# danspeech/danspeech

Measured on AMD Instinct MI355X. Metric: audio-seconds/sec (RTFx) recognize() on 10 s clips, batch=32, higher is better.
Workload: dtype f32 (two-term fp16 split operands, 3 MFMA products, fp32 accumulate)

## Files before the change

danspeech_amd/csrc/conv1_split.hip:

```cpp
#include "common.h"
#include <algorithm>

namespace dsmi {

namespace {

using f16x8 = __attribute__((ext_vector_type(8))) _Float16;
using f16x4 = __attribute__((ext_vector_type(4))) _Float16;
using f16x2 = __attribute__((ext_vector_type(2))) _Float16;
using u32x4 = __attribute__((ext_vector_type(4))) unsigned int;
constexpr float kLoScale = 2048.f, kLoInv = 1.f / 2048.f;

constexpr int KF = 41, KT = 11, SF = 2, ST = 2, PF = 20, PT = 5, CO = 32;
constexpr int C1NF = 8;
constexpr int C1NT = C1NF * 64;
constexpr int C1TT = 64;
constexpr int ROWS = SF * (C1NF - 1) + KF;
constexpr int WIN = ST * (C1TT - 1) + KT + 5;
constexpr int PITCH = 144;
constexpr int COPY = ROWS * PITCH;
constexpr size_t C1_LDS = (size_t)2 * 2 * COPY * 2;

struct Conv1Args {
    const float* x; const uint16_t* wp; const float* bias; const float* bn_a; const float* bn_b; const int32_t* out_lens;
    float* y; uint16_t* y_sp;
    int B, fi, fo, ti, to, xs, ys;
    unsigned* tile_cnt;
};

template <bool SPLIT_OUT, bool BY_DEMAND = false>
__global__ __launch_bounds__(C1NT, 4) void conv1_f16x3_kernel(Conv1Args p) {
    extern __shared__ __attribute__((aligned(16))) unsigned char c1sm[];
    _Float16* Xs = reinterpret_cast<_Float16*>(c1sm);
    const int tid0 = threadIdx.x;
    const int wv = __builtin_amdgcn_readfirstlane(tid0 >> 6);
    const ConvGrid grid{(p.to + C1TT - 1) / C1TT, (p.fo + C1NF - 1) / C1NF, p.B};
    const int total = conv_total(grid);
    const int label = blockIdx.x & 7;
    volatile int* const tk_lds = reinterpret_cast<volatile int*>(c1sm + C1_LDS);
    auto cnt_add = [&](int l) { return __hip_atomic_fetch_add(p.tile_cnt + l * kDenseCntStride, 1u, __ATOMIC_RELAXED, __HIP_MEMORY_SCOPE_AGENT); };
    auto cnt_peek = [&](int l) { return __hip_atomic_load(p.tile_cnt + l * kDenseCntStride, __ATOMIC_RELAXED, __HIP_MEMORY_SCOPE_AGENT); };
    unsigned dead = 0;
    if (BY_DEMAND) {
        if (tid0 == 0) tk_lds[0] = dense_draw(total, label, dead, cnt_add, cnt_peek, grid.nf);
        __syncthreads();
    }
  for (;;) {
    int tid = tid0;
    if (BY_DEMAND) asm volatile("" : "+v"(tid));
    const int lane = tid & 63, li = lane & 31, hk = lane >> 5;
    ConvTile tile;
    if (BY_DEMAND) {
        const int idx = __builtin_amdgcn_readfirstlane(tk_lds[0]);
        if (idx < 0) break;
        tile = conv_tile_at(grid, idx);
    } else {
        tile = ConvTile{(int)blockIdx.x, (int)blockIdx.y, (int)blockIdx.z};
    }
    const int t0 = tile.tt * C1TT, f0 = tile.ft * C1NF, b = tile.z;
    const int f = f0 + wv;
    const int olen = p.out_lens[b];
    const float *bias = p.bias, *bn_a = p.bn_a, *bn_b = p.bn_b;
    if (BY_DEMAND) asm volatile("" : "+s"(bias), "+s"(bn_a), "+s"(bn_b));
    bool own_asked = false;
    unsigned own_ticket = 0;
    auto ask = [&] { if (BY_DEMAND && tid == 0 && !((dead >> label) & 1u)) { own_asked = true; own_ticket = cnt_add(label); } };

    if (t0 >= olen) {
        ask();
        if (SPLIT_OUT) {
            for (int idx = tid; idx < C1NF * 2 * C1TT * 4; idx += C1NT) {
                const int part = idx & 3, tl = (idx >> 2) % C1TT, pl = (idx / (4 * C1TT)) % 2, ff = idx / (4 * C1TT * 2);
                if (f0 + ff < p.fo && t0 + tl < p.to)
                    *reinterpret_cast<u32x4*>(reinterpret_cast<_Float16*>(p.y_sp) + ((((size_t)b * p.fo + f0 + ff) * 2 + pl) * p.to + t0 + tl) * 32 + part * 8) = u32x4{0, 0, 0, 0};
            }
        } else {
            for (int idx = tid; idx < CO * C1NF * C1TT; idx += C1NT) {
                const int tl = idx % C1TT, ff = (idx / C1TT) % C1NF, co = idx / (C1TT * C1NF);
                if (f0 + ff < p.fo && t0 + tl < p.to) p.y[(((size_t)b * CO + co) * p.fo + f0 + ff) * p.ys + t0 + tl] = 0.f;
            }
        }
        if (BY_DEMAND) __syncthreads();
    } else {
    const int fin0 = SF * f0 - PF, tin0 = ST * t0 - PT;
    const int nlive = min(C1NF, p.fo - f0);
    const int row_lo = max(0, -fin0), row_hi = min(SF * (nlive - 1) + KF - 1, p.fi - 1 - fin0);
    for (int idx = tid + row_lo * (PITCH / 2); idx < (row_hi + 1) * (PITCH / 2); idx += C1NT) {
        const int row = idx / (PITCH / 2), q = 2 * (idx - row * (PITCH / 2));
        const int fin = fin0 + row;
        float v[2] = {0.f, 0.f};
        {
            const float* src = p.x + ((size_t)b * p.fi + fin) * p.xs;
#pragma unroll
            for (int e = 0; e < 2; ++e) {
                const int tin = tin0 + q + e;
                if (tin >= 0 && tin < p.ti && q + e < WIN) v[e] = src[tin];
            }
        }
        f16x2 h, l;
#pragma unroll
        for (int e = 0; e < 2; ++e) {
            const _Float16 hi = (_Float16)v[e];
            h[e] = hi; l[e] = (_Float16)((v[e] - (float)hi) * kLoScale);
        }
        _Float16* r0 = Xs + row * PITCH + q;
        *reinterpret_cast<f16x2*>(r0) = h;
        *reinterpret_cast<f16x2*>(r0 + 2 * COPY) = l;
        if (q >= 2) {
            *reinterpret_cast<f16x2*>(r0 + COPY - 2) = h;
            *reinterpret_cast<f16x2*>(r0 + 3 * COPY - 2) = l;
        }
    }
    __syncthreads();
    if (f < p.fo) {
    const ConvRows myr = conv_rows_of(f, p.fi, KF, PF, SF);

    f32x16 acc[2], acl[2];
#pragma unroll
    for (int tt = 0; tt < 2; ++tt)
#pragma unroll
        for (int r = 0; r < 16; ++r) { acc[tt][r] = 0.f; acl[tt][r] = 0.f; }

    const _Float16* xb = Xs + (SF * wv) * PITCH + 4 * li + 8 * hk;
    const u32x4* wq = reinterpret_cast<const u32x4*>(p.wp) + lane;
    const int kfirst = min(myr.lo, KF - 1);
    u32x4 wn[2] = {wq[(size_t)kfirst * 128], wq[(size_t)kfirst * 128 + 64]};
#pragma unroll 1
    for (int kf = myr.lo; kf <= myr.hi; ++kf) {
        const f16x8 wh = __builtin_bit_cast(f16x8, wn[0]), wl = __builtin_bit_cast(f16x8, wn[1]);
        if (kf + 1 < KF) { wn[0] = wq[(size_t)(kf + 1) * 128]; wn[1] = wq[(size_t)(kf + 1) * 128 + 64]; }
        const _Float16* xr = xb + kf * PITCH;
        f16x8 xh[2], xl[2];
#pragma unroll
        for (int tt = 0; tt < 2; ++tt) {
            const f16x4 a0 = *reinterpret_cast<const f16x4*>(xr + tt * COPY), a1 = *reinterpret_cast<const f16x4*>(xr + tt * COPY + 4);
            const f16x4 b0 = *reinterpret_cast<const f16x4*>(xr + (2 + tt) * COPY), b1 = *reinterpret_cast<const f16x4*>(xr + (2 + tt) * COPY + 4);
            xh[tt] = f16x8{a0[0], a0[1], a0[2], a0[3], a1[0], a1[1], a1[2], a1[3]};
            xl[tt] = f16x8{b0[0], b0[1], b0[2], b0[3], b1[0], b1[1], b1[2], b1[3]};
        }
#pragma unroll
        for (int tt = 0; tt < 2; ++tt) acl[tt] = __builtin_amdgcn_mfma_f32_32x32x16_f16(wl, xh[tt], acl[tt], 0, 0, 0);
#pragma unroll
        for (int tt = 0; tt < 2; ++tt) acc[tt] = __builtin_amdgcn_mfma_f32_32x32x16_f16(wh, xh[tt], acc[tt], 0, 0, 0);
#pragma unroll
        for (int tt = 0; tt < 2; ++tt) acl[tt] = __builtin_amdgcn_mfma_f32_32x32x16_f16(wh, xl[tt], acl[tt], 0, 0, 0);
    }

    ask();
#pragma unroll
    for (int tt = 0; tt < 2; ++tt) {
        const int t = t0 + 2 * li + tt;
        if (t >= p.to) continue;
        if (SPLIT_OUT) {
#pragma unroll
            for (int g = 0; g < 4; ++g) {
                f16x4 h, l;
#pragma unroll
                for (int q = 0; q < 4; ++q) {
                    const int co = q + 8 * g + 4 * hk;
                    float v = (acc[tt][4 * g + q] + acl[tt][4 * g + q] * kLoInv + bias[co]) * bn_a[co] + bn_b[co];
                    v = fminf(fmaxf(v, 0.f), 20.f);
                    v = t < olen ? v : 0.f;
                    const _Float16 a = (_Float16)v;
                    h[q] = a; l[q] = (_Float16)(v - (float)a);
                }
                _Float16* base = reinterpret_cast<_Float16*>(p.y_sp) + ((((size_t)b * p.fo + f) * 2) * (size_t)p.to + t) * 32 + 8 * g + 4 * hk;
                *reinterpret_cast<f16x4*>(base) = h;
                *reinterpret_cast<f16x4*>(base + (size_t)p.to * 32) = l;
            }
        } else {
#pragma unroll
            for (int r = 0; r < 16; ++r) {
                const int co = (r & 3) + 8 * (r >> 2) + 4 * hk;
                float v = (acc[tt][r] + acl[tt][r] * kLoInv + bias[co]) * bn_a[co] + bn_b[co];
                v = fminf(fmaxf(v, 0.f), 20.f);
                p.y[(((size_t)b * CO + co) * p.fo + f) * p.ys + t] = t < olen ? v : 0.f;
            }
        }
    }
    }
    }
    if (!BY_DEMAND) break;
    if (tid == 0) {
        int idx = own_asked ? dense_redeem(total, label, own_ticket, dead, grid.nf) : -1;
        if (idx < 0) idx = dense_steal(total, dead, cnt_add, cnt_peek, grid.nf);
        tk_lds[0] = idx;
    }
    __syncthreads();
  }
    if (BY_DEMAND && tid0 == 0) {
        unsigned* const done = p.tile_cnt + kDenseLabels * kDenseCntStride;
        if (__hip_atomic_fetch_add(done, 1u, __ATOMIC_RELAXED, __HIP_MEMORY_SCOPE_AGENT) == gridDim.x - 1) {
#pragma unroll
            for (int l = 0; l <= kDenseLabels; ++l) __hip_atomic_store(p.tile_cnt + l * kDenseCntStride, 0u, __ATOMIC_RELAXED, __HIP_MEMORY_SCOPE_AGENT);
        }
    }
}

inline uint16_t c1_bits(_Float16 h) {
    uint16_t u;
    __builtin_memcpy(&u, &h, 2);
    return u;
}

}

std::vector<uint16_t> pack_conv1_w_split(const float* w) {
    std::vector<uint16_t> out((size_t)KF * 2 * 64 * 8, 0);
    for (int kf = 0; kf < KF; ++kf)
        for (int lane = 0; lane < 64; ++lane)
            for (int e = 0; e < 8; ++e) {
                const int co = lane & 31, kt = 8 * (lane >> 5) + e;
                if (kt >= KT) continue;
                const float x = w[((size_t)co * KF + kf) * KT + kt];
                const _Float16 h1 = (_Float16)x;
                const _Float16 h2 = (_Float16)((x - (float)h1) * kLoScale);
                const size_t base = (((size_t)kf * 2) * 64 + lane) * 8 + e;
                out[base] = c1_bits(h1); out[base + 512] = c1_bits(h2);
            }
    return out;
}

namespace {
template <auto KERN>
void conv1_lds_once() {
    static std::atomic<bool> done[kLdsOnceDevices];
    int dev = 0;
    if (hipGetDevice(&dev) != hipSuccess || dev < 0 || dev >= kLdsOnceDevices || !done[dev].load(std::memory_order_acquire)) {
        (void)hipFuncSetAttribute(reinterpret_cast<const void*>(KERN), hipFuncAttributeMaxDynamicSharedMemorySize, (int)C1_LDS + 16);
        if (dev >= 0 && dev < kLdsOnceDevices) done[dev].store(true, std::memory_order_release);
    }
}
}

int launch_conv1_split(const ConvLaunch& c, const uint16_t* wp_sp, hipStream_t s) {
    Conv1Args a{c.x, wp_sp, c.bias, c.bn_a, c.bn_b, c.out_lens_dev, c.y, c.y_sp, c.B, c.fi, c.fo, c.ti, c.to, c.xs, c.ys,
                c.n_cus > 0 ? c.tile_cnt : nullptr};
    const ConvGrid g{ceil_div(c.to, C1TT), ceil_div(c.fo, C1NF), c.B};
    if (a.tile_cnt) {
        const dim3 gridd(std::min(conv_total(g), 2 * c.n_cus));
        const size_t lds = C1_LDS + 16;
        if (c.y_sp) { conv1_lds_once<conv1_f16x3_kernel<true, true>>(); DSMI_LAUNCH((conv1_f16x3_kernel<true, true>), gridd, dim3(C1NT), lds, s, c.ev, a); }
        else { conv1_lds_once<conv1_f16x3_kernel<false, true>>(); DSMI_LAUNCH((conv1_f16x3_kernel<false, true>), gridd, dim3(C1NT), lds, s, c.ev, a); }
        return (int)gridd.x;
    }
    const dim3 grid(g.nt, g.nf, g.nz);
    if (c.y_sp) { conv1_lds_once<conv1_f16x3_kernel<true>>(); DSMI_LAUNCH(conv1_f16x3_kernel<true>, grid, dim3(C1NT), C1_LDS, s, c.ev, a); }
    else { conv1_lds_once<conv1_f16x3_kernel<false>>(); DSMI_LAUNCH(conv1_f16x3_kernel<false>, grid, dim3(C1NT), C1_LDS, s, c.ev, a); }
    return g.nt * g.nf * g.nz;
}

}
```

Measured before the change: 63040.

## Repack conv1 taps into dense MFMA K groups with a weight prefetch ring

Conv1 used to spend one set of MFMAs per filter row, with only 11 of the 16 K slots holding real taps. The new layout splits each row's taps: taps 0-7 of two rows go into one main group, and taps 8-10 of four rows go into one tail group. This cuts the MFMA issue count by about a quarter and removes the padded work. Weights are repacked to match and are fetched through buffer loads into a 3-deep register ring, replacing the old one-ahead prefetch. The LDS staging grows by a few extra rows. The change adds more complex LDS read addressing and higher register pressure from the ring.

Measured after the change: 63440, median of 6. Within noise of the previous version (+0.6%).

```diff
diff --git a/danspeech_amd/csrc/conv1_split.hip b/danspeech_amd/csrc/conv1_split.hip
--- a/danspeech_amd/csrc/conv1_split.hip
+++ b/danspeech_amd/csrc/conv1_split.hip
@@ -1,4 +1,5 @@
 #include "common.h"
+#include "conv1_taps.h"
 #include <algorithm>
 
 namespace dsmi {
@@ -11,15 +12,25 @@
 using u32x4 = __attribute__((ext_vector_type(4))) unsigned int;
 constexpr float kLoScale = 2048.f, kLoInv = 1.f / 2048.f;
 
-constexpr int KF = 41, KT = 11, SF = 2, ST = 2, PF = 20, PT = 5, CO = 32;
-constexpr int C1NF = 8;
+constexpr int KF = kC1KF, KT = kC1KT, SF = kC1SF, ST = 2, PF = kC1PF, PT = 5, CO = 32;
+constexpr int C1NF = kC1NF;
 constexpr int C1NT = C1NF * 64;
 constexpr int C1TT = 64;
-constexpr int ROWS = SF * (C1NF - 1) + KF;
-constexpr int WIN = ST * (C1TT - 1) + KT + 5;
-constexpr int PITCH = 144;
+constexpr int ROWS = kC1Rows;
+constexpr int WIN = kC1Win;
+constexpr int PITCH = kC1Pitch;
+static_assert(WIN == ST * (C1TT - 1) + KT + 5, "the window of a 64-step tile");
 constexpr int COPY = ROWS * PITCH;
 constexpr size_t C1_LDS = (size_t)2 * 2 * COPY * 2;
+#ifndef DSMI_C1_WRING
+#define DSMI_C1_WRING 3
+#endif
+#if defined(DSMI_EXPERIMENTS) && defined(DSMI_C1_SKIP)
+constexpr bool C1_SKIP_STAGE = DSMI_C1_SKIP == 1, C1_SKIP_FETCH = DSMI_C1_SKIP == 2;
+#else
+constexpr bool C1_SKIP_STAGE = false, C1_SKIP_FETCH = false;
+#endif
+constexpr int C1WR = DSMI_C1_WRING;
 
 struct Conv1Args {
     const float* x; const uint16_t* wp; const float* bias; const float* bn_a; const float* bn_b; const int32_t* out_lens;
@@ -48,17 +59,20 @@
   for (;;) {
     int tid = tid0;
     if (BY_DEMAND) asm volatile("" : "+v"(tid));
+    int total_t = total;
+    ConvGrid grid_t = grid;
+    if (BY_DEMAND) asm volatile("" : "+s"(total_t), "+s"(grid_t.nf), "+s"(grid_t.nz));
     const int lane = tid & 63, li = lane & 31, hk = lane >> 5;
     ConvTile tile;
     if (BY_DEMAND) {
         const int idx = __builtin_amdgcn_readfirstlane(tk_lds[0]);
         if (idx < 0) break;
-        tile = conv_tile_at(grid, idx);
+        tile = conv_tile_at(grid_t, idx);
     } else {
         tile = ConvTile{(int)blockIdx.x, (int)blockIdx.y, (int)blockIdx.z};
     }
     const int t0 = tile.tt * C1TT, f0 = tile.ft * C1NF, b = tile.z;
-    const int f = f0 + wv;
+    const int f = __builtin_amdgcn_readfirstlane(f0 + wv);
     const int olen = p.out_lens[b];
     const float *bias = p.bias, *bn_a = p.bn_a, *bn_b = p.bn_b;
     if (BY_DEMAND) asm volatile("" : "+s"(bias), "+s"(bn_a), "+s"(bn_b));
@@ -83,13 +97,12 @@
         if (BY_DEMAND) __syncthreads();
     } else {
     const int fin0 = SF * f0 - PF, tin0 = ST * t0 - PT;
-    const int nlive = min(C1NF, p.fo - f0);
-    const int row_lo = max(0, -fin0), row_hi = min(SF * (nlive - 1) + KF - 1, p.fi - 1 - fin0);
-    for (int idx = tid + row_lo * (PITCH / 2); idx < (row_hi + 1) * (PITCH / 2); idx += C1NT) {
+    const ConvRows st = c1_staged_rows(f0, min(C1NF, p.fo - f0), p.fi);
+    for (int idx = tid + st.lo * (PITCH / 2); idx < (C1_SKIP_STAGE ? 0 : (st.hi + 1) * (PITCH / 2)); idx += C1NT) {
         const int row = idx / (PITCH / 2), q = 2 * (idx - row * (PITCH / 2));
         const int fin = fin0 + row;
         float v[2] = {0.f, 0.f};
-        {
+        if (fin < p.fi) {
             const float* src = p.x + ((size_t)b * p.fi + fin) * p.xs;
 #pragma unroll
             for (int e = 0; e < 2; ++e) {
@@ -121,29 +134,48 @@
 #pragma unroll
         for (int r = 0; r < 16; ++r) { acc[tt][r] = 0.f; acl[tt][r] = 0.f; }
 
-    const _Float16* xb = Xs + (SF * wv) * PITCH + 4 * li + 8 * hk;
-    const u32x4* wq = reinterpret_cast<const u32x4*>(p.wp) + lane;
-    const int kfirst = min(myr.lo, KF - 1);
-    u32x4 wn[2] = {wq[(size_t)kfirst * 128], wq[(size_t)kfirst * 128 + 64]};
+    const int xmain = (SF * wv + c1_read(C1Group{false, 0}, hk, 0).row) * PITCH + 4 * li;
+    const int xtail = (SF * wv + c1_read(C1Group{true, 0}, hk, 0).row) * PITCH + 4 * li + c1_read(C1Group{true, 0}, hk, 0).idx;
+    const __amdgpu_buffer_rsrc_t wq = __builtin_amdgcn_make_buffer_rsrc((void*)p.wp, 0, kC1Entries * 2048, 0x00020000);
+    const unsigned woff = 16u * lane;
+    const int ngroups = c1_main_groups(myr) + c1_tail_groups(myr);
+    u32x4 wr[C1WR][2];
+    const int glast = max(ngroups - 1, 0);
+    auto wfetch = [&](int g, u32x4 (&w)[2]) {
+        const int e = c1_entry(c1_group(myr, min(g, glast))) * 2048;
+        w[0] = __builtin_bit_cast(u32x4, __builtin_amdgcn_raw_buffer_load_b128(wq, woff, e, 0));
+        w[1] = __builtin_bit_cast(u32x4, __builtin_amdgcn_raw_buffer_load_b128(wq, woff + 1024u, e, 0));
+    };
+#pragma unroll
+    for (int s = 0; s < C1WR - 1; ++s) { wfetch(s, wr[s]); __builtin_amdgcn_sched_barrier(0); }
 #pragma unroll 1
-    for (int kf = myr.lo; kf <= myr.hi; ++kf) {
-        const f16x8 wh = __builtin_bit_cast(f16x8, wn[0]), wl = __builtin_bit_cast(f16x8, wn[1]);
-        if (kf + 1 < KF) { wn[0] = wq[(size_t)(kf + 1) * 128]; wn[1] = wq[(size_t)(kf + 1) * 128 + 64]; }
-        const _Float16* xr = xb + kf * PITCH;
-        f16x8 xh[2], xl[2];
-#pragma unroll
-        for (int tt = 0; tt < 2; ++tt) {
-            const f16x4 a0 = *reinterpret_cast<const f16x4*>(xr + tt * COPY), a1 = *reinterpret_cast<const f16x4*>(xr + tt * COPY + 4);
-            const f16x4 b0 = *reinterpret_cast<const f16x4*>(xr + (2 + tt) * COPY), b1 = *reinterpret_cast<const f16x4*>(xr + (2 + tt) * COPY + 4);
-            xh[tt] = f16x8{a0[0], a0[1], a0[2], a0[3], a1[0], a1[1], a1[2], a1[3]};
-            xl[tt] = f16x8{b0[0], b0[1], b0[2], b0[3], b1[0], b1[1], b1[2], b1[3]};
-        }
-#pragma unroll
-        for (int tt = 0; tt < 2; ++tt) acl[tt] = __builtin_amdgcn_mfma_f32_32x32x16_f16(wl, xh[tt], acl[tt], 0, 0, 0);
-#pragma unroll
-        for (int tt = 0; tt < 2; ++tt) acc[tt] = __builtin_amdgcn_mfma_f32_32x32x16_f16(wh, xh[tt], acc[tt], 0, 0, 0);
-#pragma unroll
-        for (int tt = 0; tt < 2; ++tt) acl[tt] = __builtin_amdgcn_mfma_f32_32x32x16_f16(wh, xl[tt], acl[tt], 0, 0, 0);
+    for (int g0 = 0; g0 < ngroups; g0 += C1WR) {
+#pragma unroll
+        for (int s = 0; s < C1WR; ++s) {
+            const int g = g0 + s;
+            if (g >= ngroups) break;
+            if (!C1_SKIP_FETCH) wfetch(g + C1WR - 1, wr[(s + C1WR - 1) % C1WR]);
+            __builtin_amdgcn_sched_barrier(0);
+            const C1Group q = c1_group(myr, g);
+            const _Float16* x0 = Xs + (q.tail ? xtail : xmain) + q.kf * PITCH;
+            const C1Read r0 = c1_read(q, 0, 0), r1 = c1_read(q, 0, 1);
+            const _Float16* x1 = x0 + (r1.row - r0.row) * PITCH + (r1.idx - r0.idx);
+            f16x8 xh[2], xl[2];
+#pragma unroll
+            for (int tt = 0; tt < 2; ++tt) {
+                const f16x4 a0 = *reinterpret_cast<const f16x4*>(x0 + tt * COPY), a1 = *reinterpret_cast<const f16x4*>(x1 + tt * COPY);
+                const f16x4 b0 = *reinterpret_cast<const f16x4*>(x0 + (2 + tt) * COPY), b1 = *reinterpret_cast<const f16x4*>(x1 + (2 + tt) * COPY);
+                xh[tt] = f16x8{a0[0], a0[1], a0[2], a0[3], a1[0], a1[1], a1[2], a1[3]};
+                xl[tt] = f16x8{b0[0], b0[1], b0[2], b0[3], b1[0], b1[1], b1[2], b1[3]};
+            }
+            const f16x8 wh = __builtin_bit_cast(f16x8, wr[s][0]), wl = __builtin_bit_cast(f16x8, wr[s][1]);
+#pragma unroll
+            for (int tt = 0; tt < 2; ++tt) acl[tt] = __builtin_amdgcn_mfma_f32_32x32x16_f16(wl, xh[tt], acl[tt], 0, 0, 0);
+#pragma unroll
+            for (int tt = 0; tt < 2; ++tt) acc[tt] = __builtin_amdgcn_mfma_f32_32x32x16_f16(wh, xh[tt], acc[tt], 0, 0, 0);
+#pragma unroll
+            for (int tt = 0; tt < 2; ++tt) acl[tt] = __builtin_amdgcn_mfma_f32_32x32x16_f16(wh, xl[tt], acl[tt], 0, 0, 0);
+        }
     }
 
     ask();
@@ -182,8 +214,8 @@
     }
     if (!BY_DEMAND) break;
     if (tid == 0) {
-        int idx = own_asked ? dense_redeem(total, label, own_ticket, dead, grid.nf) : -1;
-        if (idx < 0) idx = dense_steal(total, dead, cnt_add, cnt_peek, grid.nf);
+        int idx = own_asked ? dense_redeem(total_t, label, own_ticket, dead, grid_t.nf) : -1;
+        if (idx < 0) idx = dense_steal(total_t, dead, cnt_add, cnt_peek, grid_t.nf);
         tk_lds[0] = idx;
     }
     __syncthreads();
@@ -206,18 +238,14 @@
 }
 
 std::vector<uint16_t> pack_conv1_w_split(const float* w) {
-    std::vector<uint16_t> out((size_t)KF * 2 * 64 * 8, 0);
-    for (int kf = 0; kf < KF; ++kf)
-        for (int lane = 0; lane < 64; ++lane)
-            for (int e = 0; e < 8; ++e) {
-                const int co = lane & 31, kt = 8 * (lane >> 5) + e;
-                if (kt >= KT) continue;
-                const float x = w[((size_t)co * KF + kf) * KT + kt];
-                const _Float16 h1 = (_Float16)x;
-                const _Float16 h2 = (_Float16)((x - (float)h1) * kLoScale);
-                const size_t base = (((size_t)kf * 2) * 64 + lane) * 8 + e;
-                out[base] = c1_bits(h1); out[base + 512] = c1_bits(h2);
-            }
+    std::vector<uint16_t> out((size_t)kC1Entries * 2 * 64 * 8, 0);
+    c1_pack_walk([&](int entry, int lane, int e, int row, int tap) {
+        const float x = w[((size_t)(lane & 31) * KF + row) * KT + tap];
+        const _Float16 h1 = (_Float16)x;
+        const _Float16 h2 = (_Float16)((x - (float)h1) * kLoScale);
+        const size_t base = (((size_t)entry * 2) * 64 + lane) * 8 + e;
+        out[base] = c1_bits(h1); out[base + 512] = c1_bits(h2);
+    });
     return out;
 }
 
diff --git a/danspeech_amd/csrc/conv1_taps.h b/danspeech_amd/csrc/conv1_taps.h
--- /dev/null
+++ b/danspeech_amd/csrc/conv1_taps.h
@@ -0,0 +1,70 @@
+#pragma once
+
+#include "conv_rows.h"
+
+namespace dsmi {
+
+constexpr int kC1KF = 41, kC1KT = 11, kC1SF = 2, kC1PF = 20;
+constexpr int kC1NF = 8;
+constexpr int kC1Anchors = (kC1KF + 1) / 2;
+constexpr int kC1Entries = 2 * kC1Anchors;
+constexpr int kC1Rows = kC1SF * (kC1NF - 1) + kC1KF + 3;
+
+constexpr int kC1Win = 2 * 63 + 16;
+constexpr int kC1Pitch = 144;
+
+DSMI_TILES_HD inline int c1_rows_n(const ConvRows& r) { return r.hi >= r.lo ? r.hi - r.lo + 1 : 0; }
+DSMI_TILES_HD inline int c1_main_groups(const ConvRows& r) { return (c1_rows_n(r) + 1) / 2; }
+DSMI_TILES_HD inline int c1_tail_groups(const ConvRows& r) { return (c1_rows_n(r) + 3) / 4; }
+
+struct C1Group { bool tail; int kf; };
+DSMI_TILES_HD inline C1Group c1_group(const ConvRows& r, int g) {
+    const int nm = c1_main_groups(r);
+    C1Group q;
+    q.tail = g >= nm;
+    q.kf = q.tail ? r.lo + 4 * (g - nm) : r.lo + 2 * g;
+    return q;
+}
+DSMI_TILES_HD inline int c1_entry(const C1Group& q) { return (q.tail ? kC1Anchors : 0) + (q.kf >> 1); }
+
+struct C1Slot { int row, tap; };
+DSMI_TILES_HD inline C1Slot c1_slot(const C1Group& q, int hk, int e) {
+    C1Slot s;
+    if (q.tail) { s.row = q.kf + 2 * hk + (e >> 2); s.tap = 8 + (e & 3); }
+    else { s.row = q.kf + hk; s.tap = e; }
+    return s;
+}
+DSMI_TILES_HD inline bool c1_slot_real(const C1Slot& s) { return s.row < kC1KF && s.tap < kC1KT; }
+
+template <class Put>
+inline void c1_pack_walk(Put put) {
+    for (int tail = 0; tail < 2; ++tail)
+        for (int kf = 0; kf < kC1KF; kf += 2) {
+            const C1Group q{tail != 0, kf};
+            for (int lane = 0; lane < 64; ++lane)
+                for (int e = 0; e < 8; ++e) {
+                    const C1Slot sl = c1_slot(q, lane >> 5, e);
+                    if (c1_slot_real(sl)) put(c1_entry(q), lane, e, sl.row, sl.tap);
+                }
+        }
+}
+
+struct C1Read { int row, idx; };
+DSMI_TILES_HD inline C1Read c1_read(const C1Group& q, int hk, int h) {
+    C1Read a;
+    if (q.tail) { a.row = q.kf + 2 * hk + h; a.idx = 8; }
+    else { a.row = q.kf + hk; a.idx = 4 * h; }
+    return a;
+}
+
+DSMI_TILES_HD inline ConvRows c1_staged_rows(int f0, int nlive, int fi) {
+    const int fin0 = kC1SF * f0 - kC1PF;
+    const int a = kC1SF * (nlive - 1) + kC1KF - 1, b = fi - 1 - fin0;
+    ConvRows r;
+    r.lo = fin0 < 0 ? -fin0 : 0;
+    r.hi = (a < b ? a : b) + 3;
+    if (r.hi > kC1Rows - 1) r.hi = kC1Rows - 1;
+    return r;
+}
+
+}
```
